# autonomousvision/LaRa

Measured on NVIDIA B200. Metric: rasterizer fwd+bwd views/sec at 131072 Gaussians x 512x512, higher is better.
Workload: dtype f32

## Files before the change

include/surfel_rasterizer.h:

```cpp
#ifndef SURFEL_RASTERIZER_H_
#define SURFEL_RASTERIZER_H_

#include <stddef.h>
#include <stdint.h>

#ifdef __cplusplus
extern "C" {
#endif

#define SRF_ABI_VERSION 3

typedef void* srf_stream_t;

int srf_abi_version(void);
const char* srf_last_error(void);

int srf_geom_state_bytes(int P, size_t* bytes);
int srf_tile_state_bytes(int H, int W, size_t* bytes);
int srf_image_state_bytes(int H, int W, size_t* bytes);
int srf_binning_bytes(size_t capacity, size_t* entries_bytes, size_t* point_list_bytes);
int srf_backward_scratch_bytes(int P, size_t* bytes);

int srf_state_layout(int P, int H, int W, size_t geom_off[3], size_t tile_off[5], size_t image_off[2]);

int srf_forward_preprocess(srf_stream_t stream, int P, int D, int M,
// ... 116 lines not shown
```

lara_b200/_lib.py:

```python
from __future__ import annotations

import ctypes
import os
from ctypes import POINTER, c_char_p, c_float, c_int, c_size_t, c_void_p

HERE = os.path.dirname(os.path.abspath(__file__))
LIB_PATH = os.path.join(HERE, "libsurfel_b200.so")
ABI_VERSION = 3
CAM_FLOATS, CAM_VIEW, CAM_CAMPOS, CAM_BG = 24, 0, 16, 19

_P = c_void_p
SIGNATURES = {
    "srf_abi_version": (c_int, []),
    "srf_last_error": (c_char_p, []),
    "srf_geom_state_bytes": (c_int, [c_int, POINTER(c_size_t)]),
    "srf_tile_state_bytes": (c_int, [c_int, c_int, POINTER(c_size_t)]),
    "srf_image_state_bytes": (c_int, [c_int, c_int, POINTER(c_size_t)]),
    "srf_binning_bytes": (c_int, [c_size_t, POINTER(c_size_t), POINTER(c_size_t)]),
    "srf_backward_scratch_bytes": (c_int, [c_int, POINTER(c_size_t)]),
    "srf_state_layout": (c_int, [c_int, c_int, c_int, POINTER(c_size_t), POINTER(c_size_t), POINTER(c_size_t)]),
    "srf_forward_preprocess": (c_int, [
        _P, c_int, c_int, c_int,
        _P, _P, _P,
        _P, _P, c_float,
# ... 174 lines not shown
```

lara_b200/csrc/api.cu:

```cuda
#include <cuda_runtime.h>
#include <stdarg.h>
#include <stdint.h>
#include <stdio.h>
#include <stdlib.h>
#include <string.h>

#include <atomic>
#include <mutex>
#include <vector>

#include "../../include/surfel_rasterizer.h"
#include "surfel_common.cuh"
#include "surfel_kernels.h"

namespace {

thread_local char g_err[512] = "";

int fail(const char* fmt, ...) {
    va_list ap;
    va_start(ap, fmt);
    vsnprintf(g_err, sizeof(g_err), fmt, ap);
    va_end(ap);
    return 1;
}

int cuda_fail(const char* what, cudaError_t e) {
    return fail("%s: %s", what, cudaGetErrorString(e));
}

inline size_t align_up(size_t x, size_t a = 256) { return (x + a - 1) / a * a; }

struct GeomLayout { size_t rec, depths, rects, total; };
struct TileLayout { size_t count, counters, ranges, big, order, total; int gx, gy, ntiles; };
struct ImageLayout { size_t accum, ncontrib, total; };

GeomLayout geom_layout(int P) {
    GeomLayout l;
    const size_t p = (size_t)(P > 0 ? P : 0);
    size_t o = 0;
    l.rec = o; o = align_up(o + p * SRF_REC_QUADS * sizeof(float4));
    l.depths = o; o = align_up(o + p * sizeof(float));
    l.rects = o; o = align_up(o + p * sizeof(uint2));
    l.total = o + 256;
    return l;
}
// ... 50 lines not shown
namespace srf {
void prof_start(int kernel, cudaStream_t stream) {
    if (!g_prof_on) return;
    std::lock_guard<std::mutex> lk(g_prof_mu);
    g_open[kernel] = take_event();
    cudaEventRecord(g_open[kernel], stream);
}
void prof_stop(int kernel, cudaStream_t stream) {
    if (!g_prof_on) return;
    std::lock_guard<std::mutex> lk(g_prof_mu);
    ProfSpan s; s.kernel = kernel; s.start = g_open[kernel]; s.stop = take_event();
    cudaEventRecord(s.stop, stream);
    g_spans.push_back(s);
}

constexpr int kBwdVariantDefault = 18, kBwdVariantMax = 18;
static std::atomic<int> g_bwd_variant{0};
int bwd_variant() {
    int v = g_bwd_variant.load(std::memory_order_relaxed);
    if (v == 0) {
        const char* e = getenv("SRF_BWD_VARIANT");
        const int x = e ? atoi(e) : kBwdVariantDefault;
        v = (x >= 1 && x <= kBwdVariantMax) ? x : kBwdVariantDefault;
        g_bwd_variant.store(v, std::memory_order_relaxed);
    }
    return v;
}

int sm_count() {
    static int cache[64] = {0};
    int dev = 0;
// ... 54 lines not shown
int srf_tile_state_bytes(int H, int W, size_t* bytes) {
    if (H <= 0 || W <= 0 || !bytes) return fail("srf_tile_state_bytes: bad arguments");
    *bytes = tile_layout(H, W).total;
    return 0;
}

int srf_image_state_bytes(int H, int W, size_t* bytes) {
    if (H <= 0 || W <= 0 || !bytes) return fail("srf_image_state_bytes: bad arguments");
    *bytes = image_layout(H, W).total;
    return 0;
}

int srf_binning_bytes(size_t capacity, size_t* entries_bytes, size_t* point_list_bytes) {
    if (!entries_bytes || !point_list_bytes) return fail("srf_binning_bytes: bad arguments");
    *entries_bytes = align_up(capacity * sizeof(uint64_t)) + 256;
    *point_list_bytes = align_up(capacity * sizeof(uint32_t)) + 256;
    return 0;
}

int srf_backward_scratch_bytes(int P, size_t* bytes) {
    if (P < 0 || !bytes) return fail("srf_backward_scratch_bytes: bad arguments");
    *bytes = align_up((size_t)P * SRF_GRAD_FLOATS * sizeof(float)) + 256;
    return 0;
}

int srf_state_layout(int P, int H, int W, size_t geom_off[3], size_t tile_off[5], size_t image_off[2]) {
    if (P < 0 || H <= 0 || W <= 0) return fail("srf_state_layout: bad arguments");
    const GeomLayout g = geom_layout(P);
    const TileLayout t = tile_layout(H, W);
    const ImageLayout i = image_layout(H, W);
    if (geom_off) { geom_off[0] = g.rec; geom_off[1] = g.depths; geom_off[2] = g.rects; }
// ... 2 lines not shown
    return 0;
}

}

namespace {

struct Cams {
    const float* view;
    const float* campos;
    const float* bg;
    size_t stride;
};

size_t entries_stride_bytes(size_t capacity) { return align_up(capacity * sizeof(uint64_t)) + 256; }
size_t plist_stride_bytes(size_t capacity) { return align_up(capacity * sizeof(uint32_t)) + 256; }
size_t ggrad_stride_bytes(int P) { return align_up((size_t)P * SRF_GRAD_FLOATS * sizeof(float)) + 256; }

void fill_bin_args(srf::BinArgs& b, int V, int P, const TileLayout& tl, void* tile_state) {
    memset(&b, 0, sizeof(b));
    b.P = P; b.nviews = V; b.ntiles = tl.ntiles; b.gx = tl.gx;
    b.tile_count = at<uint32_t>(tile_state, tl.count);
    b.counters = at<uint32_t>(tile_state, tl.counters);
    b.ranges = at<uint2>(tile_state, tl.ranges);
    b.big_list = at<uint32_t>(tile_state, tl.big);
    b.tile_order = at<uint32_t>(tile_state, tl.order);
    b.tile_stride = V > 1 ? tl.total : 0;
}

int forward_preprocess_impl(const char* fn, cudaStream_t stream, int V, int P, int D, int M,
                            const float* means3D, const float* shs, const float* colors_precomp,
// ... 99 lines not shown
        e = srf::launch_bin_and_sort(b, stream);
        if (e != cudaSuccess) return cuda_fail("binning launch", e);
    }
    srf::RenderFwdArgs r;
    memset(&r, 0, sizeof(r));
    r.W = image_width; r.H = image_height; r.gx = tl.gx; r.gy = tl.gy; r.nviews = V;
    r.capacity = (uint32_t)capacity;
    r.ranges = b.ranges;
    r.tile_order = b.tile_order;
    r.point_list = point_list;
    r.rec = P > 0 ? at<float4>(geom_state, gl.rec) : nullptr;
    r.bg = background;
    r.out_color = out_color; r.out_others = out_others;
    r.accum = at<float>(image_state, il.accum);
    r.n_contrib = at<uint32_t>(image_state, il.ncontrib);
    r.geom_stride = b.geom_stride; r.tile_stride = b.tile_stride; r.plist_stride = b.plist_stride;
    r.image_stride = V > 1 ? il.total : 0;
    r.cam_stride = cam_stride;
    e = srf::launch_render_fwd(r, stream);
    if (e != cudaSuccess) return cuda_fail("render_fwd launch", e);
    return 0;
}

int backward_impl(const char* fn, cudaStream_t stream, int V, int P, int D, int M, int image_height, int image_width,
                  size_t capacity, Cams cams,
                  const float* means3D, const float* shs, int colors_were_precomputed,
                  const float* scales, const float* rotations, int transmat_was_precomputed,
                  float tan_fovx, float tan_fovy, const int* radii,
                  const void* geom_state, const void* tile_state, const uint32_t* point_list,
                  const void* image_state,
// ... 19 lines not shown

    cudaError_t e = cudaMemsetAsync(scratch, 0, V > 1 ? gstride * (size_t)V : (size_t)P * SRF_GRAD_FLOATS * sizeof(float), stream);
    if (e != cudaSuccess) return cuda_fail("memset gradient records", e);

    srf::RenderBwdArgs r;
    memset(&r, 0, sizeof(r));
    r.W = image_width; r.H = image_height; r.gx = tl.gx; r.gy = tl.gy; r.nviews = V;
    r.capacity = (uint32_t)capacity;
    r.ranges = at<uint2>(tile_state, tl.ranges);
    r.tile_order = at<uint32_t>(tile_state, tl.order);
    r.point_list = point_list;
    r.rec = at<float4>(geom_state, gl.rec);
    r.bg = cams.bg;
    r.accum = at<float>(image_state, il.accum);
    r.n_contrib = at<uint32_t>(image_state, il.ncontrib);
    r.dL_dpix = dL_dout_color;
    r.dL_dothers = dL_dout_others;
    r.ggrad = static_cast<float*>(scratch);
    if (V > 1) {
        r.geom_stride = gl.total; r.tile_stride = tl.total; r.plist_stride = plist_stride_bytes(capacity);
        r.image_stride = il.total; r.ggrad_stride = gstride;
    }
    r.cam_stride = cams.stride;
    e = srf::launch_render_bwd(r, stream);
    if (e != cudaSuccess) return cuda_fail("render_bwd launch", e);

    srf::PreprocessBwdArgs p;
    memset(&p, 0, sizeof(p));
    p.P = P; p.D = D; p.M = (shs && !colors_were_precomputed) ? M : 0; p.nviews = V;
    p.means3D = means3D; p.scales = scales; p.rotations = rotations;
// ... 326 lines not shown
```

lara_b200/csrc/render_bwd.cu:

```cuda
#include "surfel_common.cuh"
#include "surfel_kernels.h"

namespace srf {

namespace {

constexpr int kBwdGroup = 16;

__device__ __forceinline__ float rcp_fast(float x) {
    float r;
    asm("rcp.approx.ftz.f32 %0, %1;" : "=f"(r) : "f"(x));
    return r;
}

__device__ __forceinline__ void red_add_v4(float* addr, float a, float b, float c, float d) {
    asm volatile("red.global.add.v4.f32 [%0], {%1, %2, %3, %4};" ::"l"(addr), "f"(a), "f"(b), "f"(c), "f"(d) : "memory");
}

__device__ __forceinline__ f32x2 shfl_xor2(f32x2 v, int m) {
    return (f32x2)__shfl_xor_sync(0xffffffffu, (unsigned long long)v, m);
}

__device__ __forceinline__ uint32_t smem_addr(const void* p) { return (uint32_t)__cvta_generic_to_shared(p); }
__device__ __forceinline__ float4 lds_f4(uint32_t a) {
// ... 44 lines not shown
    const float rho = fminf(rho3d, rho2d);
    r.depth = r.lowpass ? Twz : Twz + fmaf(Twx, sx, Twy * sy);
    r.G = ex2_fast(rho * -0.72134752044448170f);
    const float araw = q2.w * r.G;
    r.alpha = fminf(0.99f, araw);
    r.valid = (pz != 0.0f) && !(r.depth < SRF_NEAR_F) && !(araw < 0.00392156862745098f);
    const bool near_thr = fabsf(araw - 0.00392156862745098f) < 4.0e-7f || fabsf(r.depth - SRF_NEAR_F) < 2.0e-5f ||
                          fabsf(rho3d - rho2d) <= 1.0e-5f * rho2d;
    if (near_thr && pz != 0.0f) {
        PairEval e;
        eval_pair(q0, q1, q2, pixx, pixy, e);
        r.depth = e.depth; r.G = e.G; r.alpha = e.alpha; r.lowpass = !(e.rho3d <= e.rho2d); r.valid = e.valid;
    }
}

template <int BATCH, int NW>
struct BwdSmem {
    static constexpr size_t rec = 0;
    static constexpr size_t x = rec + sizeof(float4) * SRF_REC_QUADS * BATCH;
    static constexpr size_t pixA = x + sizeof(float) * NW * 3 * kBwdGroup * 32;
    static constexpr size_t pixB = pixA + sizeof(float4) * NW * 32;
    static constexpr size_t list = pixB + sizeof(float4) * NW * 32;
    static constexpr size_t wmax = list + (size_t)NW * BATCH;
    static constexpr size_t total = wmax + sizeof(int) * 8;
};

template <int BATCH, int NW, int MINB, bool EXACT, int P2WALK, bool SMEMC, bool PREF = false, bool SADDR = false, bool PIXREG = false>
__global__ void __launch_bounds__(NW * 32, MINB) render_bwd_kernel(RenderBwdArgs a) {
    static_assert(BATCH <= 256, "hit lists are uint8");
    extern __shared__ __align__(16) unsigned char smem[];
    typedef BwdSmem<BATCH, NW> L;
    constexpr int NT = NW * 32;
    float4 (*s_rec)[BATCH] = reinterpret_cast<float4 (*)[BATCH]>(smem + L::rec);
    float4* s_pixA = reinterpret_cast<float4*>(smem + L::pixA);
    float4* s_pixB = reinterpret_cast<float4*>(smem + L::pixB);
    int* s_wmax = reinterpret_cast<int*>(smem + L::wmax);

    const int tid = threadIdx.x, lane = tid & 31, wid = tid >> 5;
    float* s_xw = reinterpret_cast<float*>(smem + L::x) + wid * (3 * kBwdGroup * 32);
    uint8_t* s_listw = reinterpret_cast<uint8_t*>(smem + L::list) + wid * BATCH;
    uint32_t sa_base = SADDR ? smem_addr(smem) : 0u;
    if (SADDR) asm volatile("" : "+r"(sa_base));
    const uint32_t sa_rec = sa_base + (uint32_t)L::rec, sa_x = sa_base + (uint32_t)(L::x + wid * (3 * kBwdGroup * 32 * sizeof(float))),
                   sa_list = sa_base + (uint32_t)(L::list + wid * BATCH);

    const int view = blockIdx.y;
    const size_t npix = (size_t)a.W * a.H;
    a.ranges = view_ptr(a.ranges, view, a.tile_stride);
    a.tile_order = view_ptr(a.tile_order, view, a.tile_stride);
    a.point_list = view_ptr(a.point_list, view, a.plist_stride);
    a.rec = view_ptr(a.rec, view, a.geom_stride);
    a.bg += (size_t)view * a.cam_stride;
    a.accum = view_ptr(a.accum, view, a.image_stride);
    a.n_contrib = view_ptr(a.n_contrib, view, a.image_stride);
    a.dL_dpix += (size_t)view * 3 * npix;
    a.dL_dothers += (size_t)view * 8 * npix;
    a.ggrad = view_ptr(a.ggrad, view, a.ggrad_stride);

    const int tile = (int)a.tile_order[blockIdx.x / (8 / NW)];
    const int gw = (int)(blockIdx.x % (8 / NW)) * NW + wid;
    const int tyi = tile / a.gx, txi = tile - tyi * a.gx;
    int lx, ly;
    tile_pixel(gw * 32 + lane, lx, ly);
    const int pxi = txi * SRF_TILE + lx, pyi = tyi * SRF_TILE + ly;
    const bool inside = pxi < a.W && pyi < a.H;
    const size_t pix = (size_t)pyi * a.W + pxi;
    const float bx0 = (float)(txi * SRF_TILE + ((gw & 1) << 3)) + 0.5f, by0 = (float)(tyi * SRF_TILE + ((gw >> 1) << 2)) + 0.5f;

    uint2 range = a.ranges[tile];
    if (range.y > a.capacity) range.y = range.x;

    const float T_final = inside ? a.accum[pix] : 0.0f;
    float T = T_final;
    const int last_contributor = inside ? (int)a.n_contrib[pix] : 0;
    const int median_contributor = inside ? (int)a.n_contrib[pix + npix] : 0;
    float dpix0 = 0.f, dpix1 = 0.f, dpix2 = 0.f;
    float dL_ddepth = 0.f, dL_daccum = 0.f, dL_dreg = 0.f, dn0 = 0.f, dn1 = 0.f, dn2 = 0.f;
    float dL_dmedian_depth = 0.f, dL_dmax_dweight = 0.f;
    float final_D = 0.f, final_D2 = 0.f;
    if (inside) {
        dpix0 = a.dL_dpix[pix]; dpix1 = a.dL_dpix[pix + npix]; dpix2 = a.dL_dpix[pix + 2 * npix];
        dL_ddepth = a.dL_dothers[pix];
        dL_daccum = a.dL_dothers[pix + npix];
        dn0 = a.dL_dothers[pix + 2 * npix];
        dn1 = a.dL_dothers[pix + 3 * npix];
// ... 43 lines not shown
                const uint32_t id = PREF ? next_id : __ldg(a.point_list + range.x + pos);
                const float4* r = a.rec + (size_t)id * SRF_REC_QUADS;
#pragma unroll
                for (int k = 0; k < SRF_REC_QUADS; ++k) s_rec[k][jt] = ldg4(r + k);
                s_rec[4][jt].w = __uint_as_float(id);
            }
        }
        if (PREF) {
            const int npos = n_eff - 1 - ((b + 1) * BATCH + tid);
            if (npos >= 0) next_id = __ldg(a.point_list + range.x + npos);
        }
        __syncthreads();
        const int cnt = min(BATCH, n_eff - b * BATCH);

        int nh = 0;
        for (int c = 0; c < cnt; c += 32) {
            const int jt = c + lane;
            bool hit = false;
            if (jt < cnt && n_eff - 1 - (b * BATCH + jt) < wmax) hit = octagon_hits(s_rec[2][jt], s_rec[5][jt], warp_rect_at(bx0, by0));
            const unsigned hits = __ballot_sync(0xffffffffu, hit);
            if (hit) s_listw[nh + __popc(hits & ((1u << lane) - 1u))] = (uint8_t)jt;
            nh += __popc(hits);
        }
        __syncwarp();

        for (int g0 = 0; g0 < nh; g0 += 32) {
            uint32_t colword;
            {
                uint32_t m = 0;
                if (g0 + lane < nh) {
                    const int j = s_listw[g0 + lane];
                    m = octagon_pixel_mask(s_rec[2][j], s_rec[5][j], warp_rect_at(bx0, by0));
                }
                colword = transpose32(m, lane);
            }
#pragma unroll 1
            for (int sub = 0; sub < 2; ++sub) {
                const int gbase = g0 + sub * kBwdGroup;
                if (gbase >= nh) break;
                const uint8_t* lst = s_listw + gbase;

                uint32_t bits = (colword >> (sub * kBwdGroup)) & 0xffffu;
                if (last_contributor == 0) bits = 0;
                uint32_t vbits = 0;
                const int iters1 = (int)__reduce_max_sync(0xffffffffu, (unsigned)__popc(bits));
                for (int it = 0; it < iters1; ++it) {
                    if (bits == 0) continue;
                    const int i = __ffs(bits) - 1;
                    bits &= bits - 1;
                    const int j = SADDR ? (int)lds_u8(sa_list + gbase + i) : (int)lst[i];
                    const int pos = n_eff - 1 - (b * BATCH + j);
                    if (pos >= last_contributor) continue;
                    PairBwd e;
                    const uint32_t sa_j = sa_rec + 16u * j;
                    if (SADDR)
                        eval_pair_bwd<EXACT>(lds_f4(sa_j), lds_f4(sa_j + 16u * BATCH), lds_f4(sa_j + 32u * BATCH), pixx, pixy, e);
                    else
                        eval_pair_bwd<EXACT>(s_rec[0][j], s_rec[1][j], s_rec[2][j], pixx, pixy, e);
                    if (!e.valid) continue;
                    const bool lowpass = e.lowpass;
                    const float4 q3 = SADDR ? lds_f4(sa_j + 48u * BATCH) : s_rec[3][j];
                    const float4 q4 = SADDR ? lds_f4(sa_j + 64u * BATCH) : s_rec[4][j];
                    const float alpha = e.alpha, c_d = e.depth;

                    const float r1ma = rcp_fast(1.0f - alpha);
                    T = T * r1ma;
                    const float w = alpha * T;
                    const f32x2 cur_c01 = pk2(q4.x, q4.y), cur_c2d = pk2(q4.z, c_d);
                    const f32x2 cur_n01 = pk2(q3.x, q3.y), cur_n2a = pk2(q3.z, 1.0f);
                    f32x2 dpix01 = r_dpix01, dpix2d = r_dpix2d, dn01 = r_dn01, dn2a = r_dn2a;
                    if (SMEMC) {
                        const float4 ua = s_pixA[tid], ub = s_pixB[tid];
                        dpix01 = pk2(ua.w, ub.x); dpix2d = pk2(ub.y, ub.z); dn01 = pk2(ua.x, ua.y); dn2a = pk2(ua.z, ub.w);
                    }
// ... 28 lines not shown
                        const uint32_t xa = sa_x + 4u * (uint32_t)(i * 32 + (lane ^ i));
                        sts_f(xa, lowpass ? -w : w);
                        sts_f(xa + 4u * kBwdGroup * 32, e.G * dL_dalpha);
                        sts_f(xa + 8u * kBwdGroup * 32, dL_dz);
                    } else {
                        float* xp = s_xw + (i * 32 + (lane ^ i));
                        xp[0] = lowpass ? -w : w;
                        xp[kBwdGroup * 32] = e.G * dL_dalpha;
                        xp[2 * kBwdGroup * 32] = dL_dz;
                    }
                    vbits |= 1u << i;
                }

                __syncwarp();

                const uint32_t tw = transpose32(vbits, lane);
                int own = p2_i;
                uint32_t word, mybits, tmask = 0u;
                bool have;
                int iters2;
                if (P2WALK == 3) {
                    const int npx = __popc(tw);
                    if (__ballot_sync(0xffffffffu, npx != 0) == 0u) continue;
                    int part = 0;
#pragma unroll
                    for (int k = 0; k < 8; ++k) {
                        const int c = __shfl_sync(0xffffffffu, npx, p2_h * 8 + k);
                        part += (int)(((uint32_t)(c + p2_i) * candM) >> 16);
                    }
                    const int lanes_needed = part + __shfl_xor_sync(0xffffffffu, part, 16);
                    const int C = __ffs(__ballot_sync(0xffffffffu, lanes_needed <= 32) & 0xffffu);
// ... 140 lines not shown
                        const float2 a4 = up2(A4), a5 = up2(A5), a6 = up2(A6), a7 = up2(A7);
                        red_add_v4(dst + 8, a4.x, a4.y, a5.x, a5.y);
                        red_add_v4(dst + 12, a6.x, a6.y, a7.x, a7.y);
                    }
                }
                __syncwarp();
            }
        }
    }
}

}

cudaError_t launch_render_bwd_v1(const RenderBwdArgs& a, cudaStream_t stream);

template <int B, int NW, int MINB, bool EXACT, int P2WALK, bool SMEMC, bool PREF = false, bool SADDR = false, bool PIXREG = false>
static cudaError_t launch_variant(const RenderBwdArgs& a, cudaStream_t stream) {
    auto k = render_bwd_kernel<B, NW, MINB, EXACT, P2WALK, SMEMC, PREF, SADDR, PIXREG>;
    cudaError_t e = cudaFuncSetAttribute(k, cudaFuncAttributeMaxDynamicSharedMemorySize, (int)BwdSmem<B, NW>::total);
    if (e != cudaSuccess) return e;
    k<<<dim3(a.gx * a.gy * (8 / NW), a.nviews), NW * 32, BwdSmem<B, NW>::total, stream>>>(a);
    return cudaSuccess;
}

cudaError_t launch_render_bwd(const RenderBwdArgs& a, cudaStream_t stream) {
    const int ntiles = a.gx * a.gy;
    if (ntiles <= 0 || a.nviews <= 0) return cudaSuccess;
    const int variant = bwd_variant();
    if (variant == 1) return launch_render_bwd_v1(a, stream);
    prof_start(K_RENDER_BWD, stream);
    cudaError_t e = cudaSuccess;
    switch (variant) {
        case 2: e = launch_variant<256, 8, 2, false, 1, false>(a, stream); break;
        case 3: e = launch_variant<160, 8, 3, false, 1, true>(a, stream); break;
        case 4: e = launch_variant<256, 8, 2, false, 0, false>(a, stream); break;
        case 5: e = launch_variant<256, 8, 2, true, 1, false>(a, stream); break;
        case 6: e = launch_variant<256, 4, 4, false, 1, false>(a, stream); break;
        case 7: e = launch_variant<256, 4, 4, false, 2, false>(a, stream); break;
        case 8: e = launch_variant<256, 8, 2, false, 2, false>(a, stream); break;
        case 9: e = launch_variant<256, 4, 4, false, 3, false>(a, stream); break;
        case 10: e = launch_variant<256, 8, 2, false, 3, false>(a, stream); break;
        case 11: e = launch_variant<128, 4, 5, false, 3, true>(a, stream); break;
        case 12: e = launch_variant<128, 4, 5, false, 3, false>(a, stream); break;
        case 13: e = launch_variant<64, 4, 6, false, 3, true>(a, stream); break;
        case 14: e = launch_variant<128, 8, 3, false, 3, true>(a, stream); break;
        case 15: e = launch_variant<128, 4, 5, false, 2, false>(a, stream); break;
        case 16: e = launch_variant<128, 4, 5, false, 3, false, true>(a, stream); break;
        case 17: e = launch_variant<128, 4, 5, false, 3, false, true, true>(a, stream); break;
        default: e = launch_variant<128, 4, 5, false, 3, false, true, true, true>(a, stream); break;
    }
    prof_stop(K_RENDER_BWD, stream);
    return e != cudaSuccess ? e : cudaGetLastError();
}

}
```

lara_b200/csrc/render_fwd.cu:

```cuda
#include "surfel_common.cuh"
#include "surfel_kernels.h"

namespace srf {

__global__ void __launch_bounds__(SRF_CTA_THREADS, 1024 / SRF_CTA_THREADS) render_fwd_kernel(RenderFwdArgs a) {
    __shared__ float4 s_rec[SRF_REC_QUADS][SRF_BATCH];
    __shared__ uint32_t s_mask[SRF_CTA_WARPS][SRF_BATCH_CHUNKS][32];
    __shared__ uint8_t s_list[SRF_CTA_WARPS][SRF_BATCH];

    const int tid = threadIdx.x;
    {
        const int view = blockIdx.y;
        const size_t npix_v = (size_t)a.W * a.H;
        a.ranges = view_ptr(a.ranges, view, a.tile_stride);
        a.tile_order = view_ptr(a.tile_order, view, a.tile_stride);
        a.point_list = view_ptr(a.point_list, view, a.plist_stride);
        a.rec = view_ptr(a.rec, view, a.geom_stride);
        a.bg += (size_t)view * a.cam_stride;
        a.accum = view_ptr(a.accum, view, a.image_stride);
        a.n_contrib = view_ptr(a.n_contrib, view, a.image_stride);
        a.out_color += (size_t)view * 3 * npix_v;
        a.out_others += (size_t)view * 8 * npix_v;
    }
    const int tile = (int)a.tile_order[blockIdx.x / SRF_CTAS_PER_TILE];
    const int gw = (int)(blockIdx.x % SRF_CTAS_PER_TILE) * SRF_CTA_WARPS + (tid >> 5);
    const int tyi = tile / a.gx, txi = tile - tyi * a.gx;
    int lx, ly;
    tile_pixel(gw * 32 + (tid & 31), lx, ly);
    const int pxi = txi * SRF_TILE + lx, pyi = tyi * SRF_TILE + ly;
    const bool inside = pxi < a.W && pyi < a.H;
    const float pixx = (float)pxi + 0.5f, pixy = (float)pyi + 0.5f;
    const int lane = tid & 31, wid = tid >> 5;
    const WarpRect wrect = make_warp_rect(txi, tyi, gw);

    uint2 range = a.ranges[tile];
    if (range.y > a.capacity) range.y = range.x;
    const int n = (int)(range.y - range.x);
    const int rounds = (n + SRF_BATCH - 1) / SRF_BATCH;

    bool done = !inside;
    float T = 1.0f;
    uint32_t contributor = 0, last_contributor = 0;
    f32x2 C01 = 0ull, C2r = 0ull, N01 = 0ull, N2D = 0ull, d12 = 0ull;
    float median_depth = 0.f, median_weight = 0.f;
    uint32_t median_contributor = 0;

    int todo = n;
    for (int b = 0; b < rounds; ++b, todo -= SRF_BATCH) {
        if (__syncthreads_count(done) == SRF_CTA_THREADS) break;
        const int progress = b * SRF_BATCH + tid;
        if (progress < n) {
            const uint32_t id = __ldg(a.point_list + range.x + progress);
            const float4* r = a.rec + (size_t)id * SRF_REC_QUADS;
#pragma unroll
            for (int k = 0; k < SRF_REC_QUADS; ++k) s_rec[k][tid] = ldg4(r + k);
        }
        __syncthreads();
        const int cnt = min(SRF_BATCH, todo);
        if (__all_sync(0xffffffffu, done)) continue;
        int nh = 0;
        for (int c0 = 0; c0 < cnt; c0 += 32) {
            const int jt = c0 + lane;
            const bool hit = (jt < cnt) && octagon_hits(s_rec[2][jt], s_rec[5][jt], wrect);
            const unsigned hits = __ballot_sync(0xffffffffu, hit);
            if (hit) s_list[wid][nh + __popc(hits & ((1u << lane) - 1u))] = (uint8_t)jt;
            nh += __popc(hits);
        }
        __syncwarp();
        const int nchunks = (nh + 31) >> 5;
        if (nchunks == 0) continue;
        for (int c = 0; c < nchunks; ++c) {
            const int h = (c << 5) + lane;
            uint32_t m = 0;
            if (h < nh) {
                const int jt = s_list[wid][h];
                m = octagon_pixel_mask(s_rec[2][jt], s_rec[5][jt], wrect);
            }
            s_mask[wid][c][lane] = transpose32(m, lane);
        }
        __syncwarp();

        int c = 0;
        uint32_t w = s_mask[wid][0][lane];
        if (done) { w = 0; c = nchunks; }
        for (;;) {
            while (w == 0 && c < nchunks - 1) { ++c; w = s_mask[wid][c][lane]; }
            const bool active = (w != 0);
            if (!__any_sync(0xffffffffu, active)) break;
            if (!active) continue;
            const int j = s_list[wid][(c << 5) + __ffs(w) - 1];
            w &= w - 1;
            contributor = (uint32_t)(b * SRF_BATCH + j + 1);
            PairEval e;
            eval_pair(s_rec[0][j], s_rec[1][j], s_rec[2][j], pixx, pixy, e);
            if (!e.valid) continue;
            const float alpha = e.alpha;
            const float test_T = fmul_(T, fadd_(1.0f, -alpha));
            if (!(test_T >= 0.0001f)) {
                done = true;
                w = 0; c = nchunks;
                continue;
            }
            const float4 q3 = s_rec[3][j];
            const float4 q4 = s_rec[4][j];
            const float depth = e.depth;
            const float A = fadd_(1.0f, -T);
            const float m = mapped_depth(depth);
            const float mm = fmul_(m, m);
            const float2 d12_ = up2(d12);
            const float err = fma_(-d12_.x, fadd_(m, m), fma_(A, mm, d12_.y));
            if (T > 0.5f) {
                median_depth = depth;
                median_weight = fmul_(T, alpha);
                median_contributor = contributor;
            }
            const f32x2 a2 = bc2(alpha), T2 = bc2(T);
            fma2_acc(C01, T2, mul2(pk2(q4.x, q4.y), a2));
            fma2_acc(C2r, T2, mul2(pk2(q4.z, err), a2));
            fma2_acc(N01, T2, mul2(pk2(q3.x, q3.y), a2));
            fma2_acc(N2D, T2, mul2(pk2(q3.z, depth), a2));
            fma2_acc(d12, T2, mul2(pk2(m, mm), a2));
            T = test_T;
            last_contributor = contributor;
        }
    }

    const float2 C01_ = up2(C01), C2r_ = up2(C2r), N01_ = up2(N01), N2D_ = up2(N2D), d12_f = up2(d12);
    const float C0 = C01_.x, C1 = C01_.y, C2 = C2r_.x, distortion = C2r_.y;
    const float N0 = N01_.x, N1 = N01_.y, N2 = N2D_.x, D = N2D_.y, dist1 = d12_f.x, dist2 = d12_f.y;
    if (inside) {
        const size_t npix = (size_t)a.W * a.H;
        const size_t pix = (size_t)pyi * a.W + pxi;
        a.accum[pix] = T;
        a.accum[pix + npix] = dist1;
        a.accum[pix + 2 * npix] = dist2;
        a.n_contrib[pix] = last_contributor;
        a.n_contrib[pix + npix] = median_contributor;
        a.out_color[pix] = fma_(__ldg(a.bg + 0), T, C0);
// ... 24 lines not shown
```

lara_b200/csrc/surfel_common.cuh:

```cuda
#pragma once
#include <cuda_fp16.h>
#include <cuda_runtime.h>
#include <stdint.h>

#define SRF_TILE 16
#define SRF_TILE_PIX 256
#define SRF_REC_QUADS 6
#define SRF_GRAD_FLOATS 20

#define SRF_G_DT 0
#define SRF_G_DOPAC 9
#define SRF_G_DNORMAL 10
#define SRF_G_DCOLOR 13
#define SRF_G_DMEAN2D 16

#define SRF_NEAR_F 0.2f

#define SRF_CTA_WARPS 8
#define SRF_CTA_THREADS (SRF_CTA_WARPS * 32)
#define SRF_BATCH SRF_CTA_THREADS
#define SRF_BATCH_CHUNKS (SRF_BATCH / 32)
#define SRF_CTAS_PER_TILE (8 / SRF_CTA_WARPS)

#define SRF_TILE_CTR_STRIDE 64
// ... 65 lines not shown
    lx = ((w & 1) << 3) + (l & 7);
    ly = ((w >> 1) << 2) + (l >> 3);
}

__device__ __forceinline__ float4 ldg4(const float4* p) { return __ldg(p); }

__device__ __forceinline__ float act_sigmoid(float x) { return __fdiv_rn(1.0f, fadd_(1.0f, expf(-x))); }
__device__ __forceinline__ float act_quat_norm(float4 q) {
    const float n = __fsqrt_rn(fadd_(fadd_(fmul_(q.x, q.x), fmul_(q.z, q.z)), fadd_(fmul_(q.y, q.y), fmul_(q.w, q.w))));
    return fmaxf(n, 1e-12f);
}

struct WarpRect {
    float xmin, xmax, ymin, ymax, umin, umax, vmin, vmax;
};
__device__ __forceinline__ WarpRect make_warp_rect(int tile_x, int tile_y, int wid) {
    WarpRect w;
    w.xmin = (float)(tile_x * SRF_TILE + ((wid & 1) << 3)) + 0.5f; w.xmax = w.xmin + 7.0f;
    w.ymin = (float)(tile_y * SRF_TILE + ((wid >> 1) << 2)) + 0.5f; w.ymax = w.ymin + 3.0f;
    w.umin = w.xmin + w.ymin; w.umax = w.xmax + w.ymax;
    w.vmin = w.xmin - w.ymax; w.vmax = w.xmax - w.ymin;
    return w;
}
__device__ __forceinline__ WarpRect warp_rect_at(float xmin, float ymin) {
    WarpRect w;
    w.xmin = xmin; w.xmax = xmin + 7.0f;
    w.ymin = ymin; w.ymax = ymin + 3.0f;
    w.umin = w.xmin + w.ymin; w.umax = w.xmax + w.ymax;
    w.vmin = w.xmin - w.ymax; w.vmax = w.xmax - w.ymin;
    return w;
}
__device__ __forceinline__ bool octagon_hits(const float4 q2, const float4 q5, const WarpRect& w) {
    const float cx = q2.y, cy = q2.z;
    const unsigned ux = __float_as_uint(q5.x), uy = __float_as_uint(q5.y), uu = __float_as_uint(q5.z), uv = __float_as_uint(q5.w);
    const float2 ex = __half22float2(*reinterpret_cast<const __half2*>(&ux));
    const float2 ey = __half22float2(*reinterpret_cast<const __half2*>(&uy));
    const float2 eu = __half22float2(*reinterpret_cast<const __half2*>(&uu));
    const float2 ev = __half22float2(*reinterpret_cast<const __half2*>(&uv));
    const float cu = cx + cy, cv = cx - cy;
    const bool out = (cx + ex.x > w.xmax) || (cx + ex.y < w.xmin) || (cy + ey.x > w.ymax) || (cy + ey.y < w.ymin) ||
                     (cu + eu.x > w.umax) || (cu + eu.y < w.umin) || (cv + ev.x > w.vmax) || (cv + ev.y < w.vmin);
    return !out;
}

#define SRF_MASK_EPS 0.0009765625f
// ... 13 lines not shown
    uint32_t mask = 0;
#pragma unroll
    for (int r = 0; r < 4; ++r) {
        const float y = (float)r;
        const float lo = fmaxf(xlo, fmaxf(ulo - y, vlo + y));
        const float hi = fminf(xhi, fminf(uhi - y, vhi + y));
        int ilo = __float2int_ru(lo), ihi = __float2int_rd(hi);
        ilo = max(ilo, 0); ihi = min(ihi, 7);
        const bool ok = (ilo <= ihi) && (y >= ylo) && (y <= yhi);
        const uint32_t row = ok ? ((2u << ihi) - (1u << ilo)) : 0u;
        mask |= row << (8 * r);
    }
    return mask;
}

__device__ __forceinline__ uint32_t transpose32(uint32_t x, int lane) {
    const unsigned full = 0xffffffffu;
    uint32_t y;
    y = __shfl_xor_sync(full, x, 16); x = (lane & 16) ? ((x & 0xffff0000u) | (y >> 16)) : ((x & 0x0000ffffu) | (y << 16));
    y = __shfl_xor_sync(full, x, 8);  x = (lane & 8) ? ((x & 0xff00ff00u) | ((y & 0xff00ff00u) >> 8)) : ((x & 0x00ff00ffu) | ((y & 0x00ff00ffu) << 8));
    y = __shfl_xor_sync(full, x, 4);  x = (lane & 4) ? ((x & 0xf0f0f0f0u) | ((y & 0xf0f0f0f0u) >> 4)) : ((x & 0x0f0f0f0fu) | ((y & 0x0f0f0f0fu) << 4));
    y = __shfl_xor_sync(full, x, 2);  x = (lane & 2) ? ((x & 0xccccccccu) | ((y & 0xccccccccu) >> 2)) : ((x & 0x33333333u) | ((y & 0x33333333u) << 2));
    y = __shfl_xor_sync(full, x, 1);  x = (lane & 1) ? ((x & 0xaaaaaaaau) | ((y & 0xaaaaaaaau) >> 1)) : ((x & 0x55555555u) | ((y & 0x55555555u) << 1));
    return x;
}
```

lara_b200/csrc/surfel_kernels.h:

```cpp
#pragma once
#include <cuda_runtime.h>
#include <stdint.h>
#include <stdio.h>

namespace srf {

template <typename T>
__host__ __device__ __forceinline__ T* view_ptr(T* p, int v, size_t stride_bytes) {
    return reinterpret_cast<T*>(reinterpret_cast<uintptr_t>(p) + (size_t)v * stride_bytes);
}

struct PreprocessArgs {
    int P, D, M;
    int nviews;
    const float* means3D;
    const float* scales;
    const float* rotations;
    const float* opacities;
    const float* shs;
    const float* transMat_precomp;
    const float* colors_precomp;
    const float* viewmatrix;
    const float* campos;
    size_t cam_stride;
// ... 31 lines not shown
};

struct RenderFwdArgs {
    int W, H, gx, gy;
    int nviews;
    uint32_t capacity;
    const uint2* ranges;
    const uint32_t* tile_order;
    const uint32_t* point_list;
    const float4* rec;
    const float* bg;
    float* out_color;
    float* out_others;
    float* accum;
    uint32_t* n_contrib;
    size_t geom_stride, tile_stride, plist_stride, image_stride, cam_stride;
};

struct RenderBwdArgs {
    int W, H, gx, gy;
    int nviews;
    uint32_t capacity;
    const uint2* ranges;
    const uint32_t* tile_order;
    const uint32_t* point_list;
    const float4* rec;
    const float* bg;
    const float* accum;
    const uint32_t* n_contrib;
    const float* dL_dpix;
    const float* dL_dothers;
    float* ggrad;
    size_t geom_stride, tile_stride, plist_stride, image_stride, cam_stride, ggrad_stride;
};

struct PreprocessBwdArgs {
    int P, D, M;
    int nviews;
    const float* means3D;
    const float* scales;
    const float* rotations;
    const float* shs;
    const float* viewmatrix;
    const float* campos;
// ... 94 lines not shown
```

lara_b200/debug.py:

```python
from __future__ import annotations

from typing import Dict

import torch

from . import _lib
from .rasterizer import ForwardState


class _View:

    def __init__(self, state: ForwardState, view: int):
        V = state.nviews
        def cut(t):
            n = t.numel() // V
            return t[view * n:(view + 1) * n]
        self.geom, self.tile, self.image, self.point_list = cut(state.geom), cut(state.tile), cut(state.image), cut(state.point_list)
        self.num_rendered = state.resolve()[view]


def unpack_state(state: ForwardState, P: int, H: int, W: int, view: int = 0) -> Dict[str, torch.Tensor]:
    if state.nviews > 1:
        state = _View(state, view)
    lib = _lib.load()
    g_off, t_off, i_off = _lib.layout(lib, P, H, W)
    gx, gy = (W + 15) // 16, (H + 15) // 16
    ntiles = gx * gy
    npix = H * W
    R = state.num_rendered
    out: Dict[str, torch.Tensor] = {}
    if P > 0:
        rec = state.geom[g_off[0]:g_off[0] + 96 * P].view(torch.float32).view(P, 24)
        out["rec"] = rec
# ... 4 lines not shown
        out["depths_rec"] = rec[:, 15]
        out["rgb"] = rec[:, 16:19]
        out["clamp_bits"] = rec[:, 19].view(torch.int32)
        out["depths"] = state.geom[g_off[1]:g_off[1] + 4 * P].view(torch.float32)
        rects = state.geom[g_off[2]:g_off[2] + 8 * P].view(torch.int32).view(P, 2)
        out["rect"] = torch.stack([rects[:, 0] & 0xFFFF, (rects[:, 0] >> 16) & 0xFFFF,
                                   rects[:, 1] & 0xFFFF, (rects[:, 1] >> 16) & 0xFFFF], dim=1)
        out["tiles_touched"] = (out["rect"][:, 2] - out["rect"][:, 0]) * (out["rect"][:, 3] - out["rect"][:, 1])
    out["tile_count"] = state.tile[t_off[0]:t_off[0] + 256 * ntiles].view(torch.int32).view(ntiles, 64)[:, 0]
    out["counters"] = state.tile[t_off[1]:t_off[1] + 16].view(torch.int32)
    out["ranges"] = state.tile[t_off[2]:t_off[2] + 8 * ntiles].view(torch.int32).view(ntiles, 2)
    out["accum"] = state.image[i_off[0]:i_off[0] + 12 * npix].view(torch.float32).view(3, H, W)
    out["n_contrib"] = state.image[i_off[1]:i_off[1] + 8 * npix].view(torch.int32).view(2, H, W)
    out["point_list"] = state.point_list[:4 * R].view(torch.int32) if R > 0 else state.point_list[:0].view(torch.int32)
    return out
```

Before: 2273.

## Record per-pair contribution and lowpass masks in forward, replay them in backward

The forward render kernel now writes, for each warp and each splat in a batch, a 32-bit word holding which pixels actually contributed, plus a second word for which pixels used the lowpass fallback. These words are stored in an extended point_list buffer. A new default backward variant reads the stored words in place of recomputing the pixel masks, the validity checks and the last-contributor tests, and it evaluates pairs with the lowpass branch already known. The aim is to cut redundant backward work. The cost is extra global writes in forward, a larger point_list allocation, more shared memory and an ABI bump.

```diff
diff --git a/include/surfel_rasterizer.h b/include/surfel_rasterizer.h
--- a/include/surfel_rasterizer.h
+++ b/include/surfel_rasterizer.h
@@ -8,7 +8,7 @@
 extern "C" {
 #endif
 
-#define SRF_ABI_VERSION 3
+#define SRF_ABI_VERSION 4
 
 typedef void* srf_stream_t;
 
diff --git a/lara_b200/_lib.py b/lara_b200/_lib.py
--- a/lara_b200/_lib.py
+++ b/lara_b200/_lib.py
@@ -6,7 +6,7 @@
 
 HERE = os.path.dirname(os.path.abspath(__file__))
 LIB_PATH = os.path.join(HERE, "libsurfel_b200.so")
-ABI_VERSION = 3
+ABI_VERSION = 4
 CAM_FLOATS, CAM_VIEW, CAM_CAMPOS, CAM_BG = 24, 0, 16, 19
 
 _P = c_void_p
diff --git a/lara_b200/csrc/api.cu b/lara_b200/csrc/api.cu
--- a/lara_b200/csrc/api.cu
+++ b/lara_b200/csrc/api.cu
@@ -30,6 +30,12 @@
 }
 
 inline size_t align_up(size_t x, size_t a = 256) { return (x + a - 1) / a * a; }
+
+inline size_t mask_plane_bytes(size_t capacity) { return align_up(capacity * 8 * sizeof(uint32_t)); }
+inline size_t plist_stride_bytes(size_t capacity) { return align_up(capacity * sizeof(uint32_t)) + 2 * mask_plane_bytes(capacity) + 256; }
+inline uint32_t* pair_masks_of(const uint32_t* point_list, size_t capacity) {
+    return const_cast<uint32_t*>(point_list) + align_up(capacity * sizeof(uint32_t)) / sizeof(uint32_t);
+}
 
 struct GeomLayout { size_t rec, depths, rects, total; };
 struct TileLayout { size_t count, counters, ranges, big, order, total; int gx, gy, ntiles; };
@@ -110,7 +116,7 @@
     g_spans.push_back(s);
 }
 
-constexpr int kBwdVariantDefault = 18, kBwdVariantMax = 18;
+constexpr int kBwdVariantDefault = 19, kBwdVariantMax = 19;
 static std::atomic<int> g_bwd_variant{0};
 int bwd_variant() {
     int v = g_bwd_variant.load(std::memory_order_relaxed);
@@ -195,7 +201,7 @@
 int srf_binning_bytes(size_t capacity, size_t* entries_bytes, size_t* point_list_bytes) {
     if (!entries_bytes || !point_list_bytes) return fail("srf_binning_bytes: bad arguments");
     *entries_bytes = align_up(capacity * sizeof(uint64_t)) + 256;
-    *point_list_bytes = align_up(capacity * sizeof(uint32_t)) + 256;
+    *point_list_bytes = plist_stride_bytes(capacity);
     return 0;
 }
 
@@ -228,7 +234,6 @@
 };
 
 size_t entries_stride_bytes(size_t capacity) { return align_up(capacity * sizeof(uint64_t)) + 256; }
-size_t plist_stride_bytes(size_t capacity) { return align_up(capacity * sizeof(uint32_t)) + 256; }
 size_t ggrad_stride_bytes(int P) { return align_up((size_t)P * SRF_GRAD_FLOATS * sizeof(float)) + 256; }
 
 void fill_bin_args(srf::BinArgs& b, int V, int P, const TileLayout& tl, void* tile_state) {
@@ -358,6 +363,8 @@
     r.out_color = out_color; r.out_others = out_others;
     r.accum = at<float>(image_state, il.accum);
     r.n_contrib = at<uint32_t>(image_state, il.ncontrib);
+    r.pair_masks = pair_masks_of(point_list, capacity);
+    r.mask_plane = mask_plane_bytes(capacity) / sizeof(uint32_t);
     r.geom_stride = b.geom_stride; r.tile_stride = b.tile_stride; r.plist_stride = b.plist_stride;
     r.image_stride = V > 1 ? il.total : 0;
     r.cam_stride = cam_stride;
@@ -407,6 +414,8 @@
     r.bg = cams.bg;
     r.accum = at<float>(image_state, il.accum);
     r.n_contrib = at<uint32_t>(image_state, il.ncontrib);
+    r.pair_masks = pair_masks_of(point_list, capacity);
+    r.mask_plane = mask_plane_bytes(capacity) / sizeof(uint32_t);
     r.dL_dpix = dL_dout_color;
     r.dL_dothers = dL_dout_others;
     r.ggrad = static_cast<float*>(scratch);
diff --git a/lara_b200/csrc/render_bwd.cu b/lara_b200/csrc/render_bwd.cu
--- a/lara_b200/csrc/render_bwd.cu
+++ b/lara_b200/csrc/render_bwd.cu
@@ -82,22 +82,48 @@
     }
 }
 
-template <int BATCH, int NW>
+template <int BATCH, int NW, bool MASKS = false>
 struct BwdSmem {
     static constexpr size_t rec = 0;
     static constexpr size_t x = rec + sizeof(float4) * SRF_REC_QUADS * BATCH;
     static constexpr size_t pixA = x + sizeof(float) * NW * 3 * kBwdGroup * 32;
     static constexpr size_t pixB = pixA + sizeof(float4) * NW * 32;
     static constexpr size_t list = pixB + sizeof(float4) * NW * 32;
-    static constexpr size_t wmax = list + (size_t)NW * BATCH;
-    static constexpr size_t total = wmax + sizeof(int) * 8;
+    static constexpr size_t words = list + (size_t)NW * BATCH;
+    static constexpr size_t wmax = words + (MASKS ? sizeof(uint32_t) * NW * 2 * BATCH : 0);
+    static constexpr size_t wptr = wmax + sizeof(int) * 8;
+    static constexpr size_t total = wptr + sizeof(uint32_t*) * 8;
 };
 
-template <int BATCH, int NW, int MINB, bool EXACT, int P2WALK, bool SMEMC, bool PREF = false, bool SADDR = false, bool PIXREG = false>
+__device__ __forceinline__ void eval_pair_known(const float4 q0, const float4 q1, const float4 q2, const float pixx,
+                                                const float pixy, const bool lowpass, PairBwd& r) {
+    const float Twx = q1.z, Twy = q1.w, Twz = q2.x;
+    const f32x2 pix2 = pk2(pixx, pixy);
+    const float2 klx = up2(fma2(pix2, bc2(Twx), pk2(-q0.x, -q0.y)));
+    const float2 kly = up2(fma2(pix2, bc2(Twy), pk2(-q0.z, -q0.w)));
+    const float2 klz = up2(fma2(pix2, bc2(Twz), pk2(-q1.x, -q1.y)));
+    const float pz = fma_(klx.x, kly.y, -fmul_(kly.x, klx.y));
+    const float px = fma_(kly.x, klz.y, -fmul_(klz.x, kly.y));
+    const float py = fma_(klz.x, klx.y, -fmul_(klx.x, klz.y));
+    const float rpz = rcp_fast(pz);
+    const float sx = px * rpz, sy = py * rpz;
+    const float rho3d = fmaf(sx, sx, sy * sy);
+    const float2 d = up2(sub2(pk2(q2.y, q2.z), pix2));
+    const float rho2d = 2.0f * fmaf(d.x, d.x, d.y * d.y);
+    r.lowpass = lowpass;
+    r.depth = lowpass ? Twz : Twz + fmaf(Twx, sx, Twy * sy);
+    r.G = ex2_fast((lowpass ? rho2d : rho3d) * -0.72134752044448170f);
+    r.alpha = fminf(0.99f, q2.w * r.G);
+    r.valid = true;
+}
+
+template <int BATCH, int NW, int MINB, bool EXACT, int P2WALK, bool SMEMC, bool PREF = false, bool SADDR = false, bool PIXREG = false,
+          bool MASKS = false>
 __global__ void __launch_bounds__(NW * 32, MINB) render_bwd_kernel(RenderBwdArgs a) {
     static_assert(BATCH <= 256, "hit lists are uint8");
+    static_assert(!MASKS || P2WALK == 3, "the per-pair words feed the proportional phase-2 allotment");
     extern __shared__ __align__(16) unsigned char smem[];
-    typedef BwdSmem<BATCH, NW> L;
+    typedef BwdSmem<BATCH, NW, MASKS> L;
     constexpr int NT = NW * 32;
     float4 (*s_rec)[BATCH] = reinterpret_cast<float4 (*)[BATCH]>(smem + L::rec);
     float4* s_pixA = reinterpret_cast<float4*>(smem + L::pixA);
@@ -107,6 +133,8 @@
     const int tid = threadIdx.x, lane = tid & 31, wid = tid >> 5;
     float* s_xw = reinterpret_cast<float*>(smem + L::x) + wid * (3 * kBwdGroup * 32);
     uint8_t* s_listw = reinterpret_cast<uint8_t*>(smem + L::list) + wid * BATCH;
+    uint32_t* s_cw = reinterpret_cast<uint32_t*>(smem + L::words) + wid * 2 * BATCH;
+    uint32_t* s_lw = s_cw + BATCH;
     uint32_t sa_base = SADDR ? smem_addr(smem) : 0u;
     if (SADDR) asm volatile("" : "+r"(sa_base));
     const uint32_t sa_rec = sa_base + (uint32_t)L::rec, sa_x = sa_base + (uint32_t)(L::x + wid * (3 * kBwdGroup * 32 * sizeof(float))),
@@ -133,10 +161,12 @@
     const int pxi = txi * SRF_TILE + lx, pyi = tyi * SRF_TILE + ly;
     const bool inside = pxi < a.W && pyi < a.H;
     const size_t pix = (size_t)pyi * a.W + pxi;
-    const float bx0 = (float)(txi * SRF_TILE + ((gw & 1) << 3)) + 0.5f, by0 = (float)(tyi * SRF_TILE + ((gw >> 1) << 2)) + 0.5f;
+    const float bx0 = warp_block_x0(txi, gw), by0 = warp_block_y0(tyi, gw);
 
     uint2 range = a.ranges[tile];
     if (range.y > a.capacity) range.y = range.x;
+    const uint32_t** s_wptr = reinterpret_cast<const uint32_t**>(smem + L::wptr);
+    if (MASKS && lane == 0) s_wptr[wid] = view_ptr(a.pair_masks, view, a.plist_stride) + pair_word_base(range, gw);
 
     const float T_final = inside ? a.accum[pix] : 0.0f;
     float T = T_final;
@@ -210,7 +240,33 @@
         const int cnt = min(BATCH, n_eff - b * BATCH);
 
         int nh = 0;
-        for (int c = 0; c < cnt; c += 32) {
+        if (MASKS) {
+            constexpr int NC = BATCH / 32;
+            const uint32_t* words = s_wptr[wid];
+            uint32_t cwk[NC], lwk[NC];
+#pragma unroll
+            for (int k = 0; k < NC; ++k) {
+                const int jt = k * 32 + lane, pos = n_eff - 1 - (b * BATCH + jt);
+                cwk[k] = 0u; lwk[k] = 0u;
+                if (jt < cnt && pos < wmax && octagon_hits(s_rec[2][jt], s_rec[5][jt], warp_rect_at(bx0, by0))) {
+                    cwk[k] = __ldg(words + pos);
+                    lwk[k] = __ldg(words + a.mask_plane + pos);
+                }
+            }
+#pragma unroll
+            for (int k = 0; k < NC; ++k) {
+                const bool hit = cwk[k] != 0u;
+                const unsigned hits = __ballot_sync(0xffffffffu, hit);
+                if (hit) {
+                    const int at = nh + __popc(hits & ((1u << lane) - 1u));
+                    s_listw[at] = (uint8_t)(k * 32 + lane);
+                    s_cw[at] = cwk[k];
+                    s_lw[at] = lwk[k];
+                }
+                nh += __popc(hits);
+            }
+        }
+        for (int c = 0; !MASKS && c < cnt; c += 32) {
             const int jt = c + lane;
             bool hit = false;
             if (jt < cnt && n_eff - 1 - (b * BATCH + jt) < wmax) hit = octagon_hits(s_rec[2][jt], s_rec[5][jt], warp_rect_at(bx0, by0));
@@ -221,8 +277,13 @@
         __syncwarp();
 
         for (int g0 = 0; g0 < nh; g0 += 32) {
-            uint32_t colword;
-            {
+            uint32_t colword, lpword = 0u;
+            if (MASKS) {
+                uint32_t cw_mine = 0u, lw_mine = 0u;
+                if (g0 + lane < nh) { cw_mine = s_cw[g0 + lane]; lw_mine = s_lw[g0 + lane]; }
+                colword = transpose32(cw_mine, lane);
+                lpword = transpose32(lw_mine, lane);
+            } else {
                 uint32_t m = 0;
                 if (g0 + lane < nh) {
                     const int j = s_listw[g0 + lane];
@@ -237,7 +298,8 @@
                 const uint8_t* lst = s_listw + gbase;
 
                 uint32_t bits = (colword >> (sub * kBwdGroup)) & 0xffffu;
-                if (last_contributor == 0) bits = 0;
+                const uint32_t lpbits = (lpword >> (sub * kBwdGroup)) & 0xffffu;
+                if (!MASKS && last_contributor == 0) bits = 0;
                 uint32_t vbits = 0;
                 const int iters1 = (int)__reduce_max_sync(0xffffffffu, (unsigned)__popc(bits));
                 for (int it = 0; it < iters1; ++it) {
@@ -246,14 +308,20 @@
                     bits &= bits - 1;
                     const int j = SADDR ? (int)lds_u8(sa_list + gbase + i) : (int)lst[i];
                     const int pos = n_eff - 1 - (b * BATCH + j);
-                    if (pos >= last_contributor) continue;
+                    if (!MASKS && pos >= last_contributor) continue;
                     PairBwd e;
                     const uint32_t sa_j = sa_rec + 16u * j;
-                    if (SADDR)
+                    if (MASKS) {
+                        const bool lp = (lpbits >> i) & 1u;
+                        if (SADDR)
+                            eval_pair_known(lds_f4(sa_j), lds_f4(sa_j + 16u * BATCH), lds_f4(sa_j + 32u * BATCH), pixx, pixy, lp, e);
+                        else
+                            eval_pair_known(s_rec[0][j], s_rec[1][j], s_rec[2][j], pixx, pixy, lp, e);
+                    } else if (SADDR)
                         eval_pair_bwd<EXACT>(lds_f4(sa_j), lds_f4(sa_j + 16u * BATCH), lds_f4(sa_j + 32u * BATCH), pixx, pixy, e);
                     else
                         eval_pair_bwd<EXACT>(s_rec[0][j], s_rec[1][j], s_rec[2][j], pixx, pixy, e);
-                    if (!e.valid) continue;
+                    if (!MASKS && !e.valid) continue;
                     const bool lowpass = e.lowpass;
                     const float4 q3 = SADDR ? lds_f4(sa_j + 48u * BATCH) : s_rec[3][j];
                     const float4 q4 = SADDR ? lds_f4(sa_j + 64u * BATCH) : s_rec[4][j];
@@ -312,7 +380,12 @@
 
                 __syncwarp();
 
-                const uint32_t tw = transpose32(vbits, lane);
+                uint32_t tw;
+                if (MASKS) {
+                    tw = (lane < kBwdGroup && gbase + lane < nh) ? s_cw[gbase + lane] : 0u;
+                } else {
+                    tw = transpose32(vbits, lane);
+                }
                 int own = p2_i;
                 uint32_t word, mybits, tmask = 0u;
                 bool have;
@@ -483,12 +556,14 @@
 
 cudaError_t launch_render_bwd_v1(const RenderBwdArgs& a, cudaStream_t stream);
 
-template <int B, int NW, int MINB, bool EXACT, int P2WALK, bool SMEMC, bool PREF = false, bool SADDR = false, bool PIXREG = false>
+template <int B, int NW, int MINB, bool EXACT, int P2WALK, bool SMEMC, bool PREF = false, bool SADDR = false, bool PIXREG = false,
+          bool MASKS = false>
 static cudaError_t launch_variant(const RenderBwdArgs& a, cudaStream_t stream) {
-    auto k = render_bwd_kernel<B, NW, MINB, EXACT, P2WALK, SMEMC, PREF, SADDR, PIXREG>;
-    cudaError_t e = cudaFuncSetAttribute(k, cudaFuncAttributeMaxDynamicSharedMemorySize, (int)BwdSmem<B, NW>::total);
+    auto k = render_bwd_kernel<B, NW, MINB, EXACT, P2WALK, SMEMC, PREF, SADDR, PIXREG, MASKS>;
+    constexpr size_t smem = BwdSmem<B, NW, MASKS>::total;
+    cudaError_t e = cudaFuncSetAttribute(k, cudaFuncAttributeMaxDynamicSharedMemorySize, (int)smem);
     if (e != cudaSuccess) return e;
-    k<<<dim3(a.gx * a.gy * (8 / NW), a.nviews), NW * 32, BwdSmem<B, NW>::total, stream>>>(a);
+    k<<<dim3(a.gx * a.gy * (8 / NW), a.nviews), NW * 32, smem, stream>>>(a);
     return cudaSuccess;
 }
 
@@ -516,7 +591,8 @@
         case 15: e = launch_variant<128, 4, 5, false, 2, false>(a, stream); break;
         case 16: e = launch_variant<128, 4, 5, false, 3, false, true>(a, stream); break;
         case 17: e = launch_variant<128, 4, 5, false, 3, false, true, true>(a, stream); break;
-        default: e = launch_variant<128, 4, 5, false, 3, false, true, true, true>(a, stream); break;
+        case 18: e = launch_variant<128, 4, 5, false, 3, false, true, true, true>(a, stream); break;
+        default: e = launch_variant<128, 4, 5, false, 3, false, true, true, true, true>(a, stream); break;
     }
     prof_stop(K_RENDER_BWD, stream);
     return e != cudaSuccess ? e : cudaGetLastError();
diff --git a/lara_b200/csrc/render_fwd.cu b/lara_b200/csrc/render_fwd.cu
--- a/lara_b200/csrc/render_fwd.cu
+++ b/lara_b200/csrc/render_fwd.cu
@@ -6,7 +6,10 @@
 __global__ void __launch_bounds__(SRF_CTA_THREADS, 1024 / SRF_CTA_THREADS) render_fwd_kernel(RenderFwdArgs a) {
     __shared__ float4 s_rec[SRF_REC_QUADS][SRF_BATCH];
     __shared__ uint32_t s_mask[SRF_CTA_WARPS][SRF_BATCH_CHUNKS][32];
+    __shared__ uint32_t s_lowp[SRF_CTA_WARPS][SRF_BATCH_CHUNKS][32];
     __shared__ uint8_t s_list[SRF_CTA_WARPS][SRF_BATCH];
+    __shared__ uint32_t* s_words[SRF_CTA_WARPS];
+    __shared__ uint32_t s_first;
 
     const int tid = threadIdx.x;
     {
@@ -36,7 +39,8 @@
     uint2 range = a.ranges[tile];
     if (range.y > a.capacity) range.y = range.x;
     const int n = (int)(range.y - range.x);
-    const int rounds = (n + SRF_BATCH - 1) / SRF_BATCH;
+    if (tid == 0) s_first = range.x;
+    if (lane == 0) s_words[wid] = view_ptr(a.pair_masks, (int)blockIdx.y, a.plist_stride) + pair_word_base(range, gw);
 
     bool done = !inside;
     float T = 1.0f;
@@ -45,18 +49,17 @@
     float median_depth = 0.f, median_weight = 0.f;
     uint32_t median_contributor = 0;
 
-    int todo = n;
-    for (int b = 0; b < rounds; ++b, todo -= SRF_BATCH) {
+    for (int b = 0; b * SRF_BATCH < n; ++b) {
         if (__syncthreads_count(done) == SRF_CTA_THREADS) break;
         const int progress = b * SRF_BATCH + tid;
         if (progress < n) {
-            const uint32_t id = __ldg(a.point_list + range.x + progress);
+            const uint32_t id = __ldg(a.point_list + s_first + progress);
             const float4* r = a.rec + (size_t)id * SRF_REC_QUADS;
 #pragma unroll
             for (int k = 0; k < SRF_REC_QUADS; ++k) s_rec[k][tid] = ldg4(r + k);
         }
         __syncthreads();
-        const int cnt = min(SRF_BATCH, todo);
+        const int cnt = min(SRF_BATCH, n - b * SRF_BATCH);
         if (__all_sync(0xffffffffu, done)) continue;
         int nh = 0;
         for (int c0 = 0; c0 < cnt; c0 += 32) {
@@ -76,7 +79,9 @@
                 const int jt = s_list[wid][h];
                 m = octagon_pixel_mask(s_rec[2][jt], s_rec[5][jt], wrect);
             }
-            s_mask[wid][c][lane] = transpose32(m, lane);
+            const uint32_t t = transpose32(m, lane);
+            s_mask[wid][c][lane] = done ? 0u : t;
+            s_lowp[wid][c][lane] = 0u;
         }
         __syncwarp();
 
@@ -88,16 +93,22 @@
             const bool active = (w != 0);
             if (!__any_sync(0xffffffffu, active)) break;
             if (!active) continue;
-            const int j = s_list[wid][(c << 5) + __ffs(w) - 1];
+            const int hb = __ffs(w) - 1;
+            const int j = s_list[wid][(c << 5) + hb];
             w &= w - 1;
             contributor = (uint32_t)(b * SRF_BATCH + j + 1);
             PairEval e;
             eval_pair(s_rec[0][j], s_rec[1][j], s_rec[2][j], pixx, pixy, e);
-            if (!e.valid) continue;
+            if (!e.valid) {
+                s_mask[wid][c][lane] &= ~(1u << hb);
+                continue;
+            }
             const float alpha = e.alpha;
             const float test_T = fmul_(T, fadd_(1.0f, -alpha));
             if (!(test_T >= 0.0001f)) {
                 done = true;
+                s_mask[wid][c][lane] &= ~((1u << hb) | w);
+                for (int k = c + 1; k < nchunks; ++k) s_mask[wid][k][lane] = 0u;
                 w = 0; c = nchunks;
                 continue;
             }
@@ -122,6 +133,19 @@
             fma2_acc(d12, T2, mul2(pk2(m, mm), a2));
             T = test_T;
             last_contributor = contributor;
+            if (!(e.rho3d <= e.rho2d)) s_lowp[wid][c][lane] |= 1u << hb;
+        }
+        __syncwarp();
+        uint32_t* const wr = s_words[wid] + b * SRF_BATCH;
+        for (int k = 0; k < nchunks; ++k) {
+            const uint32_t cw = transpose32(s_mask[wid][k][lane], lane);
+            const uint32_t lw = transpose32(s_lowp[wid][k][lane], lane);
+            const int h = (k << 5) + lane;
+            if (h < nh) {
+                const int jt = s_list[wid][h];
+                wr[jt] = cw;
+                wr[a.mask_plane + jt] = lw;
+            }
         }
     }
 
diff --git a/lara_b200/csrc/surfel_common.cuh b/lara_b200/csrc/surfel_common.cuh
--- a/lara_b200/csrc/surfel_common.cuh
+++ b/lara_b200/csrc/surfel_common.cuh
@@ -103,14 +103,8 @@
 struct WarpRect {
     float xmin, xmax, ymin, ymax, umin, umax, vmin, vmax;
 };
-__device__ __forceinline__ WarpRect make_warp_rect(int tile_x, int tile_y, int wid) {
-    WarpRect w;
-    w.xmin = (float)(tile_x * SRF_TILE + ((wid & 1) << 3)) + 0.5f; w.xmax = w.xmin + 7.0f;
-    w.ymin = (float)(tile_y * SRF_TILE + ((wid >> 1) << 2)) + 0.5f; w.ymax = w.ymin + 3.0f;
-    w.umin = w.xmin + w.ymin; w.umax = w.xmax + w.ymax;
-    w.vmin = w.xmin - w.ymax; w.vmax = w.xmax - w.ymin;
-    return w;
-}
+__device__ __forceinline__ float warp_block_x0(int tile_x, int gw) { return (float)(tile_x * SRF_TILE + ((gw & 1) << 3)) + 0.5f; }
+__device__ __forceinline__ float warp_block_y0(int tile_y, int gw) { return (float)(tile_y * SRF_TILE + ((gw >> 1) << 2)) + 0.5f; }
 __device__ __forceinline__ WarpRect warp_rect_at(float xmin, float ymin) {
     WarpRect w;
     w.xmin = xmin; w.xmax = xmin + 7.0f;
@@ -118,6 +112,9 @@
     w.umin = w.xmin + w.ymin; w.umax = w.xmax + w.ymax;
     w.vmin = w.xmin - w.ymax; w.vmax = w.xmax - w.ymin;
     return w;
+}
+__device__ __forceinline__ WarpRect make_warp_rect(int tile_x, int tile_y, int gw) {
+    return warp_rect_at(warp_block_x0(tile_x, gw), warp_block_y0(tile_y, gw));
 }
 __device__ __forceinline__ bool octagon_hits(const float4 q2, const float4 q5, const WarpRect& w) {
     const float cx = q2.y, cy = q2.z;
@@ -161,6 +158,10 @@
     return mask;
 }
 
+__device__ __forceinline__ size_t pair_word_base(uint2 range, int gw) {
+    return 8 * (size_t)range.x + (size_t)gw * (range.y - range.x);
+}
+
 __device__ __forceinline__ uint32_t transpose32(uint32_t x, int lane) {
     const unsigned full = 0xffffffffu;
     uint32_t y;
diff --git a/lara_b200/csrc/surfel_kernels.h b/lara_b200/csrc/surfel_kernels.h
--- a/lara_b200/csrc/surfel_kernels.h
+++ b/lara_b200/csrc/surfel_kernels.h
@@ -69,6 +69,8 @@
     float* out_others;
     float* accum;
     uint32_t* n_contrib;
+    uint32_t* pair_masks;
+    size_t mask_plane;
     size_t geom_stride, tile_stride, plist_stride, image_stride, cam_stride;
 };
 
@@ -83,6 +85,8 @@
     const float* bg;
     const float* accum;
     const uint32_t* n_contrib;
+    const uint32_t* pair_masks;
+    size_t mask_plane;
     const float* dL_dpix;
     const float* dL_dothers;
     float* ggrad;
diff --git a/lara_b200/debug.py b/lara_b200/debug.py
--- a/lara_b200/debug.py
+++ b/lara_b200/debug.py
@@ -17,6 +17,7 @@
             return t[view * n:(view + 1) * n]
         self.geom, self.tile, self.image, self.point_list = cut(state.geom), cut(state.tile), cut(state.image), cut(state.point_list)
         self.num_rendered = state.resolve()[view]
+        self.capacity = state.capacity
 
 
 def unpack_state(state: ForwardState, P: int, H: int, W: int, view: int = 0) -> Dict[str, torch.Tensor]:
@@ -51,3 +52,17 @@
     out["n_contrib"] = state.image[i_off[1]:i_off[1] + 8 * npix].view(torch.int32).view(2, H, W)
     out["point_list"] = state.point_list[:4 * R].view(torch.int32) if R > 0 else state.point_list[:0].view(torch.int32)
     return out
+
+
+def _align(x: int, a: int = 256) -> int:
+    return (x + a - 1) // a * a
+
+
+def pair_masks(state: ForwardState, view: int = 0) -> Dict[str, torch.Tensor]:
+    state.resolve()
+    if state.nviews > 1:
+        state = _View(state, view)
+    cap = int(state.capacity)
+    off, plane = _align(4 * cap), _align(32 * cap)
+    words = lambda o: state.point_list[o:o + 32 * cap].view(torch.int32)
+    return {"contrib": words(off), "lowpass": words(off + plane)}
```

After: 2345, median of 6. +3.2%, better.
